# belinghy/SteppingStone

Measured on AMD Instinct MI355X. Metric: env-steps/sec (batched random-action rollout), higher is better.
Workload: dtype f32; 1 GPU; Walker3DStepperEnv-v0, 4096 envs per MI355X, curriculum 0 (flat terrain), on-device Philox U(-1,1) actions, auto-reset on; envs_total=4096, parallelism=env-shard x1, ranks=1, steps_per_launch=1000, prewarm_steps=256

## Files before the change

steppingstone_amd/csrc/ss_dynamics.hpp:

```cpp
#pragma once
#include "ss_math.hpp"
#include "ss_pair.hpp"

namespace ss {

constexpr float kH = 1.0f / 240.0f;
constexpr float kDt = 1.0f / 60.0f;
constexpr float kGrav = 9.8f;
constexpr float kPlankA = kStonePlankHalfLength, kPlankB = kStonePlankHalfWidth;
constexpr int kPgsIters = 5;
constexpr float kErp = 0.2f;
constexpr float kSlop = 0.001f;
constexpr float kVcorrMax = 2.0f;


constexpr int kWave = 64;
constexpr int kEnvsPerWave = 32;
constexpr int kLdsSlots = 40;
constexpr int kSlotsA = 20;
constexpr int kLdsC = 0;
constexpr int kLdsT = 18;
constexpr int kLdsHead = 36;
constexpr int kScalarBase = kSlotsA * kWave * 4;
constexpr int kRecWords = 9;
constexpr int kCholWords = 15 + 6;
constexpr int kHandJc = 0, kHandL0 = kHandJc + 8 * kRecWords, kHandLc = kHandL0 + kCholWords, kHandDet = 129, kHandAct = 146, kHandFloats = 158, kHandCs = kHandLc;
constexpr bool bias_offload(int helpers) { return helpers >= 3; }
constexpr bool spine_packed(int helpers) { return helpers >= 3; }
constexpr bool torques_paired(int helpers, bool kstep) { return helpers >= 3 && kstep; }
constexpr bool response_from_lds(int helpers, bool kstep) { return helpers >= 3 && kstep; }
constexpr int kHandBias = kHandJc;
static_assert(24 <= 3 * kRecWords, "biases fit the spine records' place");
constexpr int kHandRows = kHandJc + 3 * kRecWords;
constexpr int kHandRows3 = 160;
constexpr int kHandFloats3 = kHandRows3 + 40;
constexpr int kHandSlots3 = (kHandFloats3 + 3) / 4;
constexpr int hand_slots(int helpers) { return helpers >= 3 ? kHandSlots3 : (kHandFloats + 3) / 4; }
constexpr bool rows_offload(int helpers) { return helpers >= 3; }
constexpr int kHandSlots = (kHandFloats + 3) / 4;
static_assert(kLdsSlots + kHandSlots <= 80, "two helper-variant workgroups must fit the 160 KiB of a CU (16384 envs: 512 workgroups)");
static_assert(kHandRows + 40 <= kHandJc + 8 * kRecWords, "rows fit the leg records' place");
constexpr int kHandBase = kLdsSlots * kWave * 4;
constexpr int kFarWord0 = kHandLc;
constexpr int kFarBytes = (kHandBase + kFarWord0 * kWave) * 4;
static_assert(kFarBytes <= 65536, "every hand-off word beyond the offset field of the lane's own base goes through the far base");
constexpr bool hand_far(int idx) { return idx >= kFarWord0; }
constexpr int hand_far_offset(int idx) { return (idx - kFarWord0) * kWave * 4; }
constexpr int lds_bytes(int helpers) { return (kLdsSlots + hand_slots(helpers)) * kWave * 16; }
constexpr int hand_last_word(int helpers) { return hand_slots(helpers) * 4 - 1; }
static_assert(kHandFloats3 - 1 <= hand_last_word(3) && kHandFloats + 2 - 1 <= hand_last_word(1), "the words in use (one helper: + kHandOut2's two) are allocated");
static_assert(kFarBytes + (kWave - 1) * 4 + hand_far_offset(hand_last_word(1)) + 4 <= lds_bytes(1), "one helper: far base + largest word is inside the allocation");
static_assert(kFarBytes + (kWave - 1) * 4 + hand_far_offset(hand_last_word(3)) + 4 <= lds_bytes(3), "three helpers: far base + largest word is inside the allocation");
static_assert(hand_far_offset(kFarWord0) == 0 && hand_far_offset(hand_last_word(3)) < 65536 && hand_far_offset(hand_last_word(1)) < 65536,
              "every far offset fits the 16-bit offset field");
static_assert(hand_far_offset(1) - hand_far_offset(0) == 256 && hand_far_offset(hand_last_word(3)) / 256 <= 255,
              "far offsets are multiples of 256 B within ds_*2st64_b32's reach");
constexpr int NH = 12;
enum { S_ACT = 0, S_Q = 12, S_QD = 24, S_WLAM = 36, S_POS = 48, S_QUAT = 51, S_VW = 55, S_VV = 58, S_STP = 61, S_STN = 70,
       S_WKEY = 79, S_END = 80 };
static_assert(S_END <= (kLdsSlots - kSlotsA) * 4, "LDS scalar region overflow");
constexpr bool warm_in_lds(int helpers) { return helpers < 3; }
constexpr bool reset_pose_offload(int helpers, bool kstep) { return helpers >= 3 && kstep; }
constexpr int S_POSE = S_WLAM;
static_assert(!(reset_pose_offload(0, true) && warm_in_lds(0)) && !(reset_pose_offload(1, true) && warm_in_lds(1)) &&
              !(reset_pose_offload(2, true) && warm_in_lds(2)) && !(reset_pose_offload(3, true) && warm_in_lds(3)),
              "the reset pose lives where the warm-start impulses would: only a kernel that keeps those in registers has the words to spare");
static_assert(S_POSE + NH <= S_POS, "twelve words");

constexpr int kHalf[NH] = {0, 1, 2, 3, 4, 5, 6, 7, 13, 14, 15, 16};
constexpr int left_twin(int jr) { return jr < 3 ? jr : (jr < 8 ? jr + 5 : jr + 4); }
constexpr bool mirror_flips(int j) { return kAxis[j] != 1; }
__host__ __device__ constexpr float mirror_sign(int j, float m) { return mirror_flips(j) ? m : 1.f; }
__host__ __device__ constexpr float action_lane_sign(int jr, float m) {
  return jr < 3 ? mirror_sign(jr, m) : (float)kPolicySign[jr];
}
__host__ __device__ constexpr float policy_true_sign(int jr, int side) {
  return jr < 3 ? 1.f : (float)kPolicySign[jr] * ((mirror_flips(jr) && side) ? -1.f : 1.f);
}
constexpr int first_child_half(int b) {
  int r = -1;
  for (int i = 0; i < NH; ++i)
    if (kParent[kHalf[i]] == b) r = kHalf[i] + 1;
  return r;
}

#define SS_MEMBAR() asm volatile("" ::: "memory")
#if defined(__HIP_DEVICE_COMPILE__)
#define SS_WAVE_SYNC() asm volatile("" ::: "memory")
#else
#define SS_WAVE_SYNC() ss_host_wave_sync()
#endif

#if defined(SS_PROFILE_PHASES) && defined(__HIP_DEVICE_COMPILE__)
struct Prof { uint32_t t[16]; uint32_t last; };
#define SS_PROF_DECL Prof& prof,
#define SS_PROF_ARG prof,
#define SS_PROF_RAW(i) do { uint32_t _n = __builtin_amdgcn_readfirstlane((uint32_t)__builtin_amdgcn_s_memtime()); \
    prof.t[i] = __builtin_amdgcn_readfirstlane(prof.t[i] + (_n - __builtin_amdgcn_readfirstlane(prof.last))); prof.last = _n; } while (0)
#ifdef SS_PROFILE_EPILOGUE
#define SS_PROF(i) SS_PROF_RAW(0)
#define SS_PROFE(i) SS_PROF_RAW(i)
#else
#define SS_PROF(i) SS_PROF_RAW(i)
#define SS_PROFE(i) ((void)0)
#endif
#else
#define SS_PROFE(i) ((void)0)
struct Prof { int unused; };
#define SS_PROF_DECL
#define SS_PROF_ARG
#define SS_PROF(i) ((void)0)
#endif

#if defined(SS_FUZZ_SCHED) && defined(__HIP_DEVICE_COMPILE__)
__device__ __forceinline__ void ss_fuzz(uint32_t site) {
  uint32_t h = (uint32_t)__builtin_amdgcn_s_memtime() ^ (site * 0x9E3779B9u);
  h *= 0x85EBCA6Bu; h ^= h >> 13; h *= 0xC2B2AE35u; h ^= h >> 16;
  h = __builtin_amdgcn_readfirstlane(h);
  const uint32_t n = ((h >> 8) & 3u) == 0u ? (h & 255u) : (h & 15u);
#pragma unroll 1
// ... 5 lines not shown
#endif

constexpr bool cs_offload(int helpers) { return helpers >= 3; }

struct Lds {
  float* base;
  int lane;
  SSD float2& q2(int item) const { return reinterpret_cast<float2*>(base)[item * kWave + lane]; }
  SSD float& s(int idx) const { return base[kScalarBase + idx * kWave + lane]; }
  SSD float& hs(int idx) const {
#if defined(__HIP_DEVICE_COMPILE__)
    if (hand_far(idx)) {
      int off = kFarBytes + lane * 4;
      asm("" : "+v"(off));
      return *reinterpret_cast<float*>(reinterpret_cast<char*>(base) + off + hand_far_offset(idx));
    }
#endif
    return base[kHandBase + idx * kWave + lane];
  }
};

struct Stones {
  float p[3][3], nrm[3][3], tilt[3][2];
};

struct FootReport {
  int contact;
  int on_target;
  float sole[3];
};

struct Warm {
  float lam[4][3];
  int key;
};
SSD void warm_clear(Warm& w) {
#pragma unroll
  for (int k = 0; k < 4; ++k) w.lam[k][0] = w.lam[k][1] = w.lam[k][2] = 0.f;
  w.key = 0;
}

template <class T>
struct JRecT {
  T cs, sn, Uw[3], Uv[3], Dinv, u;
};
using JRec = JRecT<float>;
using JRec2 = JRecT<ssf2>;
static_assert(sizeof(JRec2) == 2 * sizeof(JRec), "a pair record is two scalar records, nothing else");
struct JointCache {
  JRec r[NH];
  Chol6 L0;
};
constexpr int half_pos(int j) { return j <= 7 ? j : j - 5; }
SSD void put_rec(const Lds& L, int k, const JRec& r) {
  L.hs(kHandJc + k * kRecWords + 0) = r.cs; L.hs(kHandJc + k * kRecWords + 1) = r.sn; L.hs(kHandJc + k * kRecWords + 2) = r.Dinv;
#pragma unroll
  for (int m = 0; m < 3; ++m) { L.hs(kHandJc + k * kRecWords + 3 + m) = r.Uw[m]; L.hs(kHandJc + k * kRecWords + 6 + m) = r.Uv[m]; }
}
SSD void get_rec(const Lds& L, int k, JRec& r) {
  r.cs = L.hs(kHandJc + k * kRecWords + 0); r.sn = L.hs(kHandJc + k * kRecWords + 1); r.Dinv = L.hs(kHandJc + k * kRecWords + 2);
#pragma unroll
  for (int m = 0; m < 3; ++m) { r.Uw[m] = L.hs(kHandJc + k * kRecWords + 3 + m); r.Uv[m] = L.hs(kHandJc + k * kRecWords + 6 + m); }
}
SSD void put_chol(const Lds& L, const Chol6& c) {
#pragma unroll
  for (int m = 0; m < 15; ++m) L.hs(kHandL0 + m) = c.l[m];
#pragma unroll
  for (int m = 0; m < 6; ++m) L.hs(kHandL0 + 15 + m) = c.di[m];
}
SSD void get_chol(const Lds& L, Chol6& c) {
#pragma unroll
  for (int i = 0; i < 15; ++i) c.l[i] = L.hs(kHandL0 + i);
#pragma unroll
  for (int i = 0; i < 6; ++i) c.di[i] = L.hs(kHandL0 + 15 + i);
}

SSD float xchg(float x) {
#if defined(__HIP_DEVICE_COMPILE__)
  return __builtin_bit_cast(float, __builtin_amdgcn_mov_dpp(__builtin_bit_cast(int, x), 0xB1, 0xF, 0xF, true));
#else
  return ss_host_xchg(x);
#endif
}
SSD uint32_t xchg_u32(uint32_t x) {
#if defined(__HIP_DEVICE_COMPILE__)
  return (uint32_t)__builtin_amdgcn_mov_dpp((int)x, 0xB1, 0xF, 0xF, true);
#else
  return __builtin_bit_cast(uint32_t, ss_host_xchg(__builtin_bit_cast(float, x)));
#endif
}
SSD int xchg_i(int x) {
#if defined(__HIP_DEVICE_COMPILE__)
  return __builtin_amdgcn_mov_dpp(x, 0xB1, 0xF, 0xF, true);
#else
  return (int)ss_host_xchg((float)x);
#endif
}
SSD SV mirror_sv(const SV& a) {
  SV o = {{-a.w[0], a.w[1], -a.w[2]}, {a.v[0], -a.v[1], a.v[2]}};
  return o;
}
SSD SV xchg_sv(const SV& a) {
  SV t;
#pragma unroll
  for (int i = 0; i < 3; ++i) { t.w[i] = xchg(a.w[i]); t.v[i] = xchg(a.v[i]); }
  return mirror_sv(t);
}
SSD ABI xchg_abi(const ABI& a) {
  ABI o;
  constexpr float sa[6] = {1.f, 1.f, 1.f, -1.f, 1.f, -1.f};
#pragma unroll
  for (int i = 0; i < 6; ++i) { o.A.m[i] = sa[i] * xchg(a.A.m[i]); o.C.m[i] = sa[i] * xchg(a.C.m[i]); }
  constexpr float sw[3] = {-1.f, 1.f, -1.f}, sv[3] = {1.f, -1.f, 1.f};
#pragma unroll
  for (int i = 0; i < 3; ++i)
#pragma unroll
// ... 309 lines not shown

template <class Model, int K>
SSD void row_moment(float (&w)[6]) {
  constexpr float cx = Model::corners[K][0], cy = Model::corners[K][1], cz = Model::corners[K][2];
  w[0] = cy * w[5] - cz * w[4];
  w[1] = cz * w[3] - cx * w[5];
  w[2] = cx * w[4] - cy * w[3];
}
template <class Model>
SSD void jacobian_rows(const DetectOut& det, const Lds& L, ssf2 (&rWp)[12][3], float (&rB)[4]) {
  const int active = det.active, cslot = det.cslot;
  const float (&Rf)[3][3] = det.Rf;
  const float (&pen)[4] = det.pen;
  static_for<0, 4>([&](auto Kc) {
    constexpr int k = decltype(Kc)::value;
    const bool on = (active >> k) & 1;
    const int sl = (cslot >> (2 * k)) & 3;
    float n[3];
#pragma unroll
    for (int i = 0; i < 3; ++i) n[i] = on ? L.s(S_STN + sl * 3 + i) : (i == 2 ? 1.f : 0.f);
    float t1[3] = {1.f - n[0] * n[0], -n[0] * n[1], -n[0] * n[2]};
    float inv = SS_RSQRT(t1[0] * t1[0] + t1[1] * t1[1] + t1[2] * t1[2]);
    t1[0] *= inv; t1[1] *= inv; t1[2] *= inv;
    float t2[3];
    cross(n, t1, t2);
    float corr = fmaxf(pen[k] - kSlop, 0.f);
    rB[k] = on ? fminf(kErp * corr * (1.0f / kH), kVcorrMax) : 0.f;
    static_for<0, 3>([&](auto Dc) {
      constexpr int d = decltype(Dc)::value, row = k * 3 + d;
      const float* dir = d == 0 ? n : (d == 1 ? t1 : t2);
      float w[6];
#pragma unroll
      for (int c = 0; c < 3; ++c) w[3 + c] = Rf[0][c] * dir[0] + Rf[1][c] * dir[1] + Rf[2][c] * dir[2];
      row_moment<Model, k>(w);
#pragma unroll
      for (int i = 0; i < 3; ++i) rWp[row][i] = ssf2{w[2 * i], w[2 * i + 1]};
    });
  });
}

template <class JT, class T>
SSD SVT<T> aba_acc(const JRecT<T>& r, const T& qd, const SVT<T>& aprev, const SVT<T>& vb, T& qdd) {
  constexpr int ax = JT::AX, ai = (ax + 1) % 3, aj = (ax + 2) % 3;
  SVT<T> a = xmotion<JT>(r.cs, r.sn, aprev);
  a.w[ai] += qd * vb.w[aj]; a.w[aj] -= qd * vb.w[ai];
  a.v[ai] += qd * vb.v[aj]; a.v[aj] -= qd * vb.v[ai];
  T dotv = r.Uw[0] * a.w[0] + r.Uw[1] * a.w[1] + r.Uw[2] * a.w[2] + r.Uv[0] * a.v[0] + r.Uv[1] * a.v[1] +
           r.Uv[2] * a.v[2];
  qdd = r.Dinv * (r.u - dotv);
  a.w[ax] += qdd;
  return a;
}

#ifndef SS_HOST_HARNESS
template <class Model, int HELPERS, int CS_PER, class Extra>
__device__ __forceinline__ void helper_substep(int helper, const Lds& L, Extra&& extra) {
  static_assert(CS_PER == 4 || CS_PER == 6, "the 12 cos / sin pairs go to three helpers (4 each) or to two (6 each)");
  __syncthreads();
  SS_FUZZ(0x10u + helper);
  if constexpr (cs_offload(HELPERS)) {
    constexpr int kIdle = HELPERS - NH / CS_PER;
    const int first = (helper - kIdle) * CS_PER;
    if (kIdle == 0 || helper >= kIdle) {
      float qh[CS_PER], c_[CS_PER], s_[CS_PER];
#pragma unroll
      for (int k = 0; k < CS_PER; ++k) qh[k] = L.s(S_Q + first + k);
      SS_MEMBAR();
#pragma unroll
      for (int k = 0; k < CS_PER; ++k) ss_sincos(qh[k], s_[k], c_[k]);
#pragma unroll
      for (int k = 0; k < CS_PER; ++k) { L.hs(kHandCs + first + k) = c_[k]; L.hs(kHandCs + NH + first + k) = s_[k]; }
    }
    __syncthreads();
    SS_FUZZ(0x20u + helper);
  }
  float rowdir[12][3], rowB[4];
  DetectOut det0;
  if (helper == 0) {
    float cs8[8], sn8[8];
    float quat[4] = {L.s(S_QUAT), L.s(S_QUAT + 1), L.s(S_QUAT + 2), L.s(S_QUAT + 3)};
    if constexpr (cs_offload(HELPERS)) {
#pragma unroll
      for (int k = 0; k < 8; ++k) { cs8[k] = L.hs(kHandCs + k); sn8[k] = L.hs(kHandCs + NH + k); }
      SS_MEMBAR();
    } else {
      float q8[8];
#pragma unroll
      for (int k = 0; k < 8; ++k) q8[k] = L.s(S_Q + k);
      SS_MEMBAR();
#pragma unroll
      for (int k = 0; k < 8; ++k) ss_sincos(q8[k], sn8[k], cs8[k]);
    }
    float Rb[3][3];
    quat_rot(quat, Rb);
    DetectOut det;
    FootReport fr;
    fk_detect<Model, (HELPERS < 3)>(cs8, sn8, Rb, L, det, fr);
    const int flags = det.active | (det.cslot << 4) | (fr.contact << 12) | (fr.on_target << 13);
    L.hs(kHandDet + 13) = __builtin_bit_cast(float, flags);
#pragma unroll
    for (int i = 0; i < 3; ++i) L.hs(kHandDet + 14 + i) = fr.sole[i];
    if constexpr (!rows_offload(HELPERS)) {
#pragma unroll
      for (int a = 0; a < 3; ++a)
#pragma unroll
        for (int c = 0; c < 3; ++c) L.hs(kHandDet + a * 3 + c) = det.Rf[a][c];
#pragma unroll
// ... 59 lines not shown
  static_for<0, 3>([&](auto Cc) {
    constexpr int c = decltype(Cc)::value;
    if (HELPERS == 1 || helper == c) {
      const LamPair lp = operator_pair_b<Model, c>(L, jc, oc[HELPERS == 1 ? c : 0]);
#pragma unroll
      for (int i = 0; i < 3; ++i) {
        L.hs(kHandLc + (2 * c) * 6 + 2 * i) = lp.a[i].x; L.hs(kHandLc + (2 * c) * 6 + 2 * i + 1) = lp.a[i].y;
        L.hs(kHandLc + (2 * c + 1) * 6 + 2 * i) = lp.b[i].x; L.hs(kHandLc + (2 * c + 1) * 6 + 2 * i + 1) = lp.b[i].y;
      }
    }
  });
  __syncthreads();
  SS_FUZZ(0x50u + helper);
}
#endif

template <class Model, int J>
SSD void joint_limit(float q, float& viol, float& kl, float& dl) {
  constexpr float lo = Model::lo[J], hi = Model::hi[J], klim = Model::klim[J], dlim = Model::dlim[J];
  static_assert(lo < hi, "a joint's range is not empty");
  viol = fminf(q - lo, 0.f) + fmaxf(q - hi, 0.f);
  uint32_t m = viol != 0.f ? 0xFFFFFFFFu : 0u;
  SS_REG(m);
  kl = __builtin_bit_cast(float, __builtin_bit_cast(uint32_t, klim) & m);
  dl = __builtin_bit_cast(float, __builtin_bit_cast(uint32_t, dlim) & m);
}

template <class Model, int J>
SSD void joint_tau(float power, float q, float qd, float act, float& tau, float& Dadd) {
  constexpr float h = kH;
  constexpr float kd = Model::damping[J], ks = Model::stiffness[J], arm = Model::armature[J], tq = Model::torque[J];
  float viol, kl, dl;
  joint_limit<Model, J>(q, viol, kl, dl);
  tau = power * tq * act - kd * qd - ks * (q + h * qd) - kl * (viol + h * qd) - dl * qd;
  Dadd = arm + h * (kd + dl) + (h * h) * (ks + kl);
}

template <class Model, int JL, int JA>
SSD void joint_tau(float power, ssf2 q, ssf2 qd, ssf2 act, ssf2& tau, ssf2& Dadd) {
  constexpr float h = kH;
  constexpr ssf2 kd = {Model::damping[JL], Model::damping[JA]}, ks = {Model::stiffness[JL], Model::stiffness[JA]};
  constexpr ssf2 arm = {Model::armature[JL], Model::armature[JA]}, tq = {Model::torque[JL], Model::torque[JA]};
  float violl, kll, dll, viola, kla, dla;
  joint_limit<Model, JL>(q.x, violl, kll, dll);
  joint_limit<Model, JA>(q.y, viola, kla, dla);
  const ssf2 viol = pkv(violl, viola), kl = pkv(kll, kla), dl = pkv(dll, dla);
  tau = power * tq * act - kd * qd - ks * (q + h * qd) - kl * (viol + h * qd) - dl * qd;
  Dadd = arm + h * (kd + dl) + (h * h) * (ks + kl);
}

template <class Model, int HELPERS = 0, bool KSTEP = false>
SSD void substep(SS_PROF_DECL float power, FootReport& fr, const Lds& L, Warm& wm) {
  constexpr float h = kH;
  JointCache jc;
#if defined(__HIP_DEVICE_COMPILE__)
  if constexpr (HELPERS > 0) { __syncthreads(); SS_FUZZ(0x1Fu); }
#endif
  SS_PROF(0);
  float qdfr[NH];
#define SS_QDF(k) qdfr[k]
  float qd_all[NH], q_all[NH], act_all[NH];
#pragma unroll
  for (int k = 0; k < NH; ++k) { q_all[k] = L.s(S_Q + k); qd_all[k] = L.s(S_QD + k); act_all[k] = L.s(S_ACT + k); }
  SS_MEMBAR();
  auto joint_tau = [&](auto Jc, float q, float qd, float act, float& tau, float& Dadd) {
    ss::joint_tau<Model, decltype(Jc)::value>(power, q, qd, act, tau, Dadd);
  };
  float tau_pre[NH], dadd_pre[NH];
  if constexpr (cs_offload(HELPERS) && HELPERS > 0) {
    static_for<0, NH>([&](auto Kc) {
      constexpr int k = decltype(Kc)::value;
      if constexpr (torques_paired(HELPERS, KSTEP) && k >= 3 && k != 7) {
        if constexpr (k < 7) {
          ssf2 tau2, dadd2;
          ss::joint_tau<Model, kHalf[k], kHalf[k + 5]>(power, pkv(q_all[k], q_all[k + 5]), pkv(qd_all[k], qd_all[k + 5]),
                                                       pkv(act_all[k], act_all[k + 5]), tau2, dadd2);
          tau_pre[k] = tau2.x; tau_pre[k + 5] = tau2.y; dadd_pre[k] = dadd2.x; dadd_pre[k + 5] = dadd2.y;
        }
      } else {
        joint_tau(std::integral_constant<int, kHalf[k]>{}, q_all[k], qd_all[k], act_all[k], tau_pre[k], dadd_pre[k]);
      }
    });
#if defined(__HIP_DEVICE_COMPILE__)
    __builtin_amdgcn_sched_barrier(0);
    SS_PROF(1);
    __syncthreads();
    SS_PROF(12);
    SS_FUZZ(0x2Fu);
    __builtin_amdgcn_sched_barrier(0);
#endif
#pragma unroll
    for (int k = 0; k < NH; ++k) { jc.r[k].cs = L.hs(kHandCs + k); jc.r[k].sn = L.hs(kHandCs + NH + k); }
    SS_MEMBAR();
  } else {
    static_for<0, NH>([&](auto Kc) {
      constexpr int k = decltype(Kc)::value;
      ss_sincos(q_all[k], jc.r[k].sn, jc.r[k].cs);
    });
  }
  auto tau_of = [&](auto Jc, auto Kc, float& tau, float& Dadd) {
    constexpr int k = decltype(Kc)::value;
    if constexpr (cs_offload(HELPERS) && HELPERS > 0) { tau = tau_pre[k]; Dadd = dadd_pre[k]; }
    else joint_tau(Jc, q_all[k], qd_all[k], act_all[k], tau, Dadd);
  };
  SS_PROF(1);

// ... 307 lines not shown
    det.cslot = (flags >> 4) & 255;
    fr.contact = (flags >> 12) & 1;
    fr.on_target = (flags >> 13) & 1;
#pragma unroll
    for (int i = 0; i < 3; ++i) fr.sole[i] = L.hs(kHandDet + 14 + i);
  } else {
    float cs8[8], sn8[8];
#pragma unroll
    for (int k = 0; k < 8; ++k) { cs8[k] = jc.r[k].cs; sn8[k] = jc.r[k].sn; }
    fk_detect<Model>(cs8, sn8, Rb, L, det, fr);
  }
  SS_PROF(6);

  float dqd[NH];
  SV dv0;
#pragma unroll
  for (int k = 0; k < NH; ++k) dqd[k] = 0.f;
#pragma unroll
  for (int i = 0; i < 3; ++i) { dv0.w[i] = 0.f; dv0.v[i] = 0.f; }
  const int active = det.active;
  const int pair_active = active | xchg_i(active);
  const bool in_contact = pair_active != 0;
  ssf2 Lc[6][3];
  SS_PROF(7);
  float V[6];
  ssf2 rWp[12][3];
  float rB[4];
  auto rows_free = [&]() {
      {
        SV a = v0f;
        static_for<0, 8>([&](auto Jc) {
          constexpr int j = decltype(Jc)::value;
          a = xmotion<Model, j>(jc.r[j].cs, jc.r[j].sn, a);
          a.w[kAxis[j]] += SS_QDF(j);
        });
#pragma unroll
        for (int i = 0; i < 3; ++i) { V[i] = a.w[i]; V[3 + i] = a.v[i]; }
      }
      if constexpr (!rows_offload(HELPERS)) jacobian_rows<Model>(det, L, rWp, rB);
      if constexpr (rows_offload(HELPERS)) {
        static_for<0, 12>([&](auto Rc) {
          constexpr int row = decltype(Rc)::value;
          float w[6];
#pragma unroll
          for (int i = 0; i < 3; ++i) w[3 + i] = L.hs(kHandRows3 + row * 3 + i);
          row_moment<Model, row / 3>(w);
#pragma unroll
          for (int i = 0; i < 3; ++i) rWp[row][i] = ssf2{w[2 * i], w[2 * i + 1]};
        });
#pragma unroll
        for (int k = 0; k < 4; ++k) rB[k] = L.hs(kHandRows3 + 36 + k);
      }
  };
  auto solve = [&]() {
      float ul[NH];
      float wlam_prev[4][3];
      int wkey_prev = 0;
      auto load_warm = [&]() {
        if constexpr (warm_in_lds(HELPERS)) {
          wkey_prev = __builtin_bit_cast(int, L.s(S_WKEY));
#pragma unroll
          for (int k = 0; k < 4; ++k)
#pragma unroll
            for (int d = 0; d < 3; ++d) wlam_prev[k][d] = L.s(S_WLAM + 3 * k + d);
        } else {
          wkey_prev = wm.key;
#pragma unroll
          for (int k = 0; k < 4; ++k)
#pragma unroll
            for (int d = 0; d < 3; ++d) wlam_prev[k][d] = wm.lam[k][d];
        }
      };
      if constexpr (HELPERS > 0) load_warm();
      if constexpr (HELPERS > 0) {
#pragma unroll
        for (int b = 0; b < 6; ++b)
#pragma unroll
          for (int i = 0; i < 3; ++i) Lc[b][i] = pkv(L.hs(kHandLc + b * 6 + 2 * i), L.hs(kHandLc + b * 6 + 2 * i + 1));
      }
      ssf2 rYp[12][3];
      float rIA[12];
      static_for<0, 12>([&](auto Rc) {
        constexpr int row = decltype(Rc)::value, k = row / 3;
        const bool on = (active >> k) & 1;
        ssf2 y[3];
#pragma unroll
        for (int i = 0; i < 3; ++i) y[i] = pk_mul_half<0>(Lc[0][i], rWp[row][0]);
        static_for<1, 6>([&](auto Bc) {
          constexpr int b = decltype(Bc)::value;
#pragma unroll
          for (int i = 0; i < 3; ++i) y[i] = pk_fma_half<b & 1>(Lc[b][i], rWp[row][b >> 1], y[i]);
        });
#pragma unroll
        for (int i = 0; i < 3; ++i) rYp[row][i] = y[i];
        ssf2 acc = rWp[row][0] * y[0];
        acc = rWp[row][1] * y[1] + acc;
        acc = rWp[row][2] * y[2] + acc;
        rIA[row] = on ? SS_RCP(acc.x + acc.y) : 0.f;
      });
      SS_PROF(8);
      if constexpr (HELPERS == 0) load_warm();
      float lam[4][3];
      const int key = active;
      int warm_any = 0;
#pragma unroll
      for (int k = 0; k < 4; ++k) {
        const bool w = ((active & wkey_prev) >> k) & 1;
        warm_any |= w ? 1 : 0;
// ... 68 lines not shown
        for (int l = 0; l < 6; ++l) {
          const float sc = (l & 1) ? dWo[l >> 1].y : dWo[l >> 1].x;
          const ssf2 s2 = {sc, sc};
#pragma unroll
          for (int i = 0; i < 3; ++i) {
            Vp[i] = Cc[l][i] * s2 + Vp[i];
          }
        }
      }
#if defined(__HIP_DEVICE_COMPILE__)
      if constexpr (response_from_lds(HELPERS, KSTEP)) {
        sweep_with([&](auto Rc) {
          constexpr int row = decltype(Rc)::value;
          if constexpr (row == 0 || row == 5 || row == 9) {
            __builtin_amdgcn_sched_barrier(0);
            if constexpr (row == 0) {
#pragma unroll
              for (int k = 7; k >= 5; --k) get_rec(L, k, jc.r[k]);
            } else if constexpr (row == 5) {
#pragma unroll
              for (int k = 4; k >= 0; --k) get_rec(L, k, jc.r[k]);
            } else {
              get_chol(L, jc.L0);
            }
            __builtin_amdgcn_sched_barrier(0);
          }
        });
      } else
#endif
      sweep();
      SV W = {{Wp[0].x, Wp[0].y, Wp[1].x}, {Wp[1].y, Wp[2].x, Wp[2].y}};
      if constexpr (warm_in_lds(HELPERS)) {
#pragma unroll
        for (int k = 0; k < 4; ++k)
#pragma unroll
          for (int d = 0; d < 3; ++d) L.s(S_WLAM + 3 * k + d) = lam[k][d];
        L.s(S_WKEY) = __builtin_bit_cast(float, key);
      } else {
#pragma unroll
        for (int k = 0; k < 4; ++k)
#pragma unroll
          for (int d = 0; d < 3; ++d) wm.lam[k][d] = lam[k][d];
        wm.key = key;
      }
      SS_PROF(9);
      {
        SV p = {{-W.w[0], -W.w[1], -W.w[2]}, {-W.v[0], -W.v[1], -W.v[2]}};
        static_rfor<7, 3>([&](auto Jc) { p = imp_up<Model, decltype(Jc)::value>(jc, ul, p); });
        const SV po = xchg_sv(p);
#pragma unroll
        for (int i = 0; i < 3; ++i) { p.w[i] += po.w[i]; p.v[i] += po.v[i]; }
        static_rfor<2, 0>([&](auto Jc) { p = imp_up<Model, decltype(Jc)::value>(jc, ul, p); });
        dv0 = chol6_solve_neg(jc.L0, p);
        SV d = dv0;
        static_for<0, 8>([&](auto Jc) {
          constexpr int j = decltype(Jc)::value;
          d = imp_down<Model, j, true>(jc, ul, d, &dqd[half_pos(j)]);
        });
        d = dv0;
        static_for<13, 17>([&](auto Jc) {
          constexpr int j = decltype(Jc)::value;
          d = imp_down<Model, j, false>(jc, ul, d, &dqd[half_pos(j)]);
        });
      }
  };
  if (!in_contact) {
    if constexpr (warm_in_lds(HELPERS)) L.s(S_WKEY) = 0.f;
    else wm.key = 0;
  }
  if constexpr (HELPERS == 0) {
    if (in_contact) {
      JointCache jo;
      operator_records_leg(jc, jo);
      operator_records_spine(jc, jo);
      static_for<0, 3>([&](auto Cc) { operator_T<Model, decltype(Cc)::value>(jo, L); });
      static_for<0, 3>([&](auto Cc) {
        constexpr int c = decltype(Cc)::value;
        OpCarry oc;
        operator_up<Model, c>(jo, oc);
        const LamPair lp = operator_pair_b<Model, c>(L, jo, oc);
#pragma unroll
        for (int i = 0; i < 3; ++i) { Lc[2 * c][i] = lp.a[i]; Lc[2 * c + 1][i] = lp.b[i]; }
      });
      rows_free();
      solve();
    }
  } else {
    if (in_contact) rows_free();
#if defined(__HIP_DEVICE_COMPILE__)
    SS_PROF(8);
    __syncthreads();
    SS_PROF(7);
    SS_FUZZ(0x5Fu);
#endif
    if (in_contact) solve();
  }
  SS_MEMBAR();
  SS_PROF(10);

  {
    float qf[NH], qq[NH];
#pragma unroll
    for (int k = 0; k < NH; ++k) { qf[k] = SS_QDF(k); qq[k] = L.s(S_Q + k); }
    SS_MEMBAR();
#pragma unroll
    for (int k = 0; k < NH; ++k) {
      float qd = qf[k] + dqd[k];
      L.s(S_QD + k) = qd;
      L.s(S_Q + k) = qq[k] + h * qd;
    }
  }
  SV v0n;
#pragma unroll
  for (int i = 0; i < 3; ++i) { v0n.w[i] = v0f.w[i] + dv0.w[i]; v0n.v[i] = v0f.v[i] + dv0.v[i]; }
#pragma unroll
  for (int i = 0; i < 3; ++i) { L.s(S_VW + i) = v0n.w[i]; L.s(S_VV + i) = v0n.v[i]; }
#pragma unroll
  for (int r = 0; r < 3; ++r)
    L.s(S_POS + r) += h * (Rb[r][0] * v0n.v[0] + Rb[r][1] * v0n.v[1] + Rb[r][2] * v0n.v[2]);
  {
    float qw = quat[0], qx = quat[1], qy = quat[2], qz = quat[3];
    float ox = v0n.w[0], oy = v0n.w[1], oz = v0n.w[2], hh = 0.5f * h;
    float nw = qw + hh * (-qx * ox - qy * oy - qz * oz);
    float nx = qx + hh * (qw * ox + qy * oz - qz * oy);
    float ny = qy + hh * (qw * oy - qx * oz + qz * ox);
    float nz = qz + hh * (qw * oz + qx * oy - qy * ox);
    float inv = SS_RSQRT(nw * nw + nx * nx + ny * ny + nz * nz);
    L.s(S_QUAT) = nw * inv; L.s(S_QUAT + 1) = nx * inv; L.s(S_QUAT + 2) = ny * inv; L.s(S_QUAT + 3) = nz * inv;
  }
  SS_MEMBAR();
  SS_PROF(11);
}

}
```

steppingstone_amd/csrc/ss_kernels.hpp:

```cpp
#pragma once
#include <cstdlib>

#include "ss_dynamics.hpp"
#include "../../include/steppingstone.h"

namespace ss {

enum { F_POS = 0, F_QUAT = 3, F_VEL = 7, F_Q = 13, F_QD = 34, F_POT = 55, F_ZINIT = 56, F_EPRET = 57, F_NNDR = 58,
       F_STONE = 59, F_HEAD = 59 + 24, F_EPRET_LO = 59 + 30, NF = 59 + 30 + 1 };
enum { I_N = 0, I_COUNT = 1, I_ELAPSED = 2, I_RNG = 3, I_FLAGS = 4, I_PROV = 5, NI = 6 };
constexpr int kNumStones = 20;
constexpr int kNumSubsteps = 4;
constexpr float kDeg = 0.017453292519943295f;

struct Knobs {
  const float* prob;
  int per_env_prob;
  int curriculum;
  float power;
  int auto_reset;
};

struct Params {
  float* fstate;
// ... 760 lines not shown
#else
      false;
#endif
  constexpr bool kPose =
#if defined(__HIP_DEVICE_COMPILE__)
      reset_pose_offload(HELPERS, ROLLOUT);
#else
      false;
#endif
  static_assert(!kPose || kOffload, "the pose's helper and the counter's hand-off word are the output stage's kernel's");
  const int e_raw = lane_global >> 1, side = lane_global & 1;
  const bool valid = e_raw < P.n;
  int e = valid ? e_raw : P.n - 1;
  const size_t np = (size_t)P.npad;
  const float m = side ? -1.f : 1.f;
  const Lds L{lds, lane};
  float ain[NH];
  load_in<!RANDOM_ACT>(P, e, RANDOM_ACT ? nullptr : io.act + (size_t)e * NJ, side, m, L, ain);

  const int nsteps = ROLLOUT ? io.nsteps : 1;
#pragma unroll 1
  for (int kstep = 0; kstep < nsteps; ++kstep) {
  SS_FUZZ(0x60u);
  if constexpr (RANDOM_ACT) {
    bool drawn = false;
    if constexpr (ROLLOUT && HELPERS > 1) {
      if (kstep > 0) {
        float a[NH];
#pragma unroll
        for (int k = 0; k < NH; ++k) a[k] = L.hs(kHandAct + k);
#pragma unroll
        for (int k = 0; k < NH; ++k) L.s(S_ACT + k) = a[k];
        drawn = true;
      }
    }
    if (!drawn) random_actions_half(P, e, side, m, (uint32_t)io.t + (uint32_t)kstep, [&](int k, float a) { L.s(S_ACT + k) = a; });
  } else {
    put_actions(L, m, ain);
  }

  const float power = P.knobs->power;
  FootReport fr;
#if defined(SS_PROFILE_PHASES) && defined(__HIP_DEVICE_COMPILE__)
  Prof prof;
#pragma unroll
  for (int i = 0; i < 16; ++i) prof.t[i] = 0;
  prof.last = (uint32_t)__builtin_amdgcn_s_memtime();
#endif
  Warm wm;
  warm_clear(wm);
  if constexpr (warm_in_lds(HELPERS)) L.s(S_WKEY) = 0.f;
#pragma unroll 1
  for (int k = 0; k < kNumSubsteps; ++k) substep<Model, HELPERS, ROLLOUT>(SS_PROF_ARG power, fr, L, wm);
  SS_FUZZ(0x61u);
  SS_PROF(12);
  SS_MEMBAR();
  SS_OPAQUE(e);
  const float* F = P.fstate + e;
  const Knobs K = *P.knobs;
  Cache c;
  load_cache(P, e, c);
  float pot_prev = F[F_POT * np], z_init = F[F_ZINIT * np];
  float ep_ret = F[F_EPRET * np], ep_lo = F[F_EPRET_LO * np], nn_dr = F[F_NNDR * np];
  int n = P.istate[e + I_N * np], count = P.istate[e + I_COUNT * np], elapsed = P.istate[e + I_ELAPSED * np];
  uint32_t ctr = (uint32_t)P.istate[e + I_RNG * np];
  const uint32_t ctr_in = ctr;
  SS_PROFE(1);

  float pos[3], quat[4];
  SV v0;
  get_base(L, m, pos, quat, v0);
  elapsed += 1;
  const float my_sole[3] = {fr.sole[0], m * fr.sole[1], fr.sole[2]};
  float ot_sole[3];
#pragma unroll
  for (int i = 0; i < 3; ++i) ot_sole[i] = xchg(my_sole[i]);
  const int ot_contact = xchg_i(fr.contact), ot_target = xchg_i(fr.on_target);
  float sole[2][3];
#pragma unroll
  for (int i = 0; i < 3; ++i) { sole[0][i] = side ? ot_sole[i] : my_sole[i]; sole[1][i] = side ? my_sole[i] : ot_sole[i]; }
  int flags = side ? (ot_contact | (fr.contact << 1)) : (fr.contact | (ot_contact << 1));
  const int on_target = fr.on_target | ot_target;
  SS_PROFE(2);
  float accv = 0.f, e_sum = 0.f, a2 = 0.f;
  int at_limit = 0;
  static_for<0, NH>([&](auto Kc) {
    constexpr int k = decltype(Kc)::value, jr = kHalf[k];
    constexpr float mid = 0.5f * (Model::lo[jr] + Model::hi[jr]);
    constexpr float span = Model::hi[jr] - Model::lo[jr];
    const float q = L.s(S_Q + k), qd = L.s(S_QD + k), a = L.s(S_ACT + k);
    const bool mine = (jr >= 3) || (side == 0);
    accv += q + qd;
    if (mine) {
      e_sum += fabsf(a * (0.1f * qd));
      a2 += a * a;
      if (fabsf(2.f * (q - mid) / span) > 0.99f) at_limit += 1;
    }
  });
  accv += pos[0] + pos[1] + pos[2] + quat[0] + quat[1] + quat[2] + quat[3];
#pragma unroll
  for (int i = 0; i < 3; ++i) accv += v0.w[i] + v0.v[i];
  e_sum += xchg(e_sum);
  a2 += xchg(a2);
  at_limit += xchg_i(at_limit);
  const bool finite = finite_bits(accv) && (xchg_i(finite_bits(accv) ? 1 : 0) != 0);
  SS_PROFE(3);
// ... 198 lines not shown
  SS_FUZZ(0x70u + wave);
  if (wave == 0) {
    step_env<Model, RANDOM_ACT, HELPERS>(P, io, blockIdx.x * kWave + lane, lane, lds);
  } else {
    const Lds L{lds, lane};
#pragma unroll 1
    for (int k = 0; k < kNumSubsteps; ++k) helper_substep<Model, HELPERS, 6>(wave - 1, L, [](int) {});
  }
}
template <class Model>
__global__ __launch_bounds__(kWave, 1) void rollout_kernel(Params P, StepIO io) {
  __shared__ float4 lds4[kLdsSlots * kWave];
  step_env<Model, true, 0, true>(P, io, blockIdx.x * kWave + threadIdx.x, threadIdx.x, reinterpret_cast<float*>(lds4));
}
template <class Model, int HELPERS>
__global__ __launch_bounds__(kWave * (1 + HELPERS), 1) void rollout_kernel_helped(Params P, StepIO io) {
  __shared__ float4 lds4[(kLdsSlots + hand_slots(HELPERS)) * kWave];
  const int wave = __builtin_amdgcn_readfirstlane(threadIdx.x >> 6), lane = threadIdx.x & (kWave - 1);
  float* lds = reinterpret_cast<float*>(lds4);
  SS_FUZZ(0x70u + wave);
  if (wave == 0) {
    step_env<Model, true, HELPERS, true>(P, io, blockIdx.x * kWave + lane, lane, lds);
  } else {
    const Lds L{lds, lane};
    const int lane_global = blockIdx.x * kWave + lane, side = lane_global & 1;
    const int e = min(lane_global >> 1, P.n - 1);
    const float m = side ? -1.f : 1.f;
    constexpr int kPoseHelper = 0;
    uint32_t ctr_pose = 0u;
    if constexpr (reset_pose_offload(HELPERS, true))
      if (wave - 1 == kPoseHelper) ctr_pose = (uint32_t)P.istate[e + I_RNG * (size_t)P.npad];
#pragma unroll 1
    for (int kstep = 0; kstep < io.nsteps; ++kstep)
#pragma unroll 1
      for (int k = 0; k < kNumSubsteps; ++k) {
        helper_substep<Model, HELPERS, 4>(wave - 1, L, [&](int helper) {
          if (k != 0) return;
          SS_FUZZ(0x80u + helper);
          constexpr int kActHelper = 1, kEmitHelper = HELPERS - 1;
          if (HELPERS > 1 && helper == kActHelper && kstep + 1 < io.nsteps)
            random_actions_half(P, e, side, m, (uint32_t)io.t + (uint32_t)kstep + 1u, [&](int j, float a) { L.hs(kHandAct + j) = a; });
          if (out_offload(HELPERS, true) && helper == kEmitHelper && kstep > 0) emit_from_handoff<Model, true>(P, io, L, lane, lane_global, kstep - 1, lds);
        });
        if constexpr (reset_pose_offload(HELPERS, true)) {
          if (k == 0 && wave - 1 == kPoseHelper) {
            SS_FUZZ(0xA0u);
            const uint32_t ctr_now = kstep == 0 ? ctr_pose : __builtin_bit_cast(uint32_t, L.hs(kHandCtr));
            if (kstep == 0 || __any(ctr_now != ctr_pose)) {
              ctr_pose = ctr_now;
              reset_pose_half<Model>(P, e, side, m, ctr_now, [&](int j, float q) { L.s(S_POSE + j) = q; });
            }
          }
        }
      }
    if constexpr (out_offload(HELPERS, true)) {
      __syncthreads();
      SS_FUZZ(0x90u + wave);
      if (wave == 2) emit_from_handoff<Model, true>(P, io, L, lane, lane_global, io.nsteps - 1, lds);
    }
  }
}

template <class Model>
SSD void reset_env(const Params& P, int e, float* obs_row) {
  const size_t np = (size_t)P.npad;
  Dyn s;
  Cache c;
  uint32_t ctr = (uint32_t)P.istate[e + I_RNG * np];
  float pot, z_init, nn_dr;
  env_reset<Model>(P, e, s, c, ctr, pot, z_init, nn_dr);
  store_dyn(P, e, s);
  store_cache(P, e, c);
  const float straight[3][2] = {{1.f, 0.f}, {1.f, 0.f}, {1.f, 0.f}};
  store_headings(P, e, straight);
  P.fstate[e + F_POT * np] = pot;
  P.fstate[e + F_ZINIT * np] = z_init;
  P.fstate[e + F_EPRET * np] = 0.f;
  P.fstate[e + F_EPRET_LO * np] = 0.f;
  P.fstate[e + F_NNDR * np] = nn_dr;
  P.istate[e + I_N * np] = 1;
  P.istate[e + I_COUNT * np] = 0;
  P.istate[e + I_ELAPSED * np] = 0;
  P.istate[e + I_RNG * np] = (int)ctr;
  P.istate[e + I_FLAGS * np] = 0;
  if (obs_row) {
    float o[SS_OBS_DIM];
    write_obs<Model>(s, z_init, 0, c, o);
#pragma unroll
    for (int i = 0; i < SS_OBS_DIM; ++i) obs_row[i] = o[i];
  }
}

template <class Model>
__global__ __launch_bounds__(kWave) void reset_kernel(Params P, float* obs) {
  const int e = blockIdx.x * kWave + threadIdx.x;
  if (e >= P.n) return;
  reset_env<Model>(P, e, obs ? obs + (size_t)e * SS_OBS_DIM : nullptr);
}

template <class Model>
__global__ __launch_bounds__(kWave) void obs_kernel(Params P, float* obs) {
  const int e = blockIdx.x * kWave + threadIdx.x;
  if (e >= P.n) return;
  const size_t np = (size_t)P.npad;
  Dyn s;
  Cache c;
// ... 51 lines not shown
```

Before: 99.36 million env-steps/s.

## Offload arm impulse response and base integration to helper waves

After the contact solve, the main wave hands off dv0, the four arm joint records and the free base velocity through LDS. Helper wave 1 then propagates the impulse down the arm chain and integrates the arm joints, while helper wave 2 integrates the base pose and velocity. This takes work off the main wave's critical path. In exchange it adds an extra __syncthreads per substep plus one after the last substep, along with LDS traffic for the handoff.

```diff
diff --git a/steppingstone_amd/csrc/ss_dynamics.hpp b/steppingstone_amd/csrc/ss_dynamics.hpp
--- a/steppingstone_amd/csrc/ss_dynamics.hpp
+++ b/steppingstone_amd/csrc/ss_dynamics.hpp
@@ -66,6 +66,19 @@
               !(reset_pose_offload(2, true) && warm_in_lds(2)) && !(reset_pose_offload(3, true) && warm_in_lds(3)),
               "the reset pose lives where the warm-start impulses would: only a kernel that keeps those in registers has the words to spare");
 static_assert(S_POSE + NH <= S_POS, "twelve words");
+#ifndef SS_ARM_TAIL
+#define SS_ARM_TAIL 1
+#endif
+#ifndef SS_BASE_TAIL
+#define SS_BASE_TAIL 1
+#endif
+constexpr bool arm_tail_offload(int helpers, bool kstep) { return SS_ARM_TAIL != 0 && helpers >= 3 && kstep; }
+constexpr bool base_tail_offload(int helpers, bool kstep) { return SS_BASE_TAIL != 0 && helpers >= 3 && kstep; }
+constexpr bool limb_tail_offload(int helpers, bool kstep) { return arm_tail_offload(helpers, kstep) || base_tail_offload(helpers, kstep); }
+constexpr int kHandArm = kHandRows3, kHandDv0 = kHandDet, kHandV0f = kHandDv0 + 6;
+constexpr int kArmHelper = 1, kBaseHelper = 2;
+static_assert(kHandArm + 4 * kRecWords <= kHandRows3 + 36, "the arm records fit the rows' directions");
+static_assert(kHandV0f + 6 <= kHandDet + 13, "dv0 and v0f stay below the detection's flags word and the sole");
 
 constexpr int kHalf[NH] = {0, 1, 2, 3, 4, 5, 6, 7, 13, 14, 15, 16};
 constexpr int left_twin(int jr) { return jr < 3 ? jr : (jr < 8 ? jr + 5 : jr + 4); }
@@ -177,16 +190,18 @@
   Chol6 L0;
 };
 constexpr int half_pos(int j) { return j <= 7 ? j : j - 5; }
-SSD void put_rec(const Lds& L, int k, const JRec& r) {
-  L.hs(kHandJc + k * kRecWords + 0) = r.cs; L.hs(kHandJc + k * kRecWords + 1) = r.sn; L.hs(kHandJc + k * kRecWords + 2) = r.Dinv;
-#pragma unroll
-  for (int m = 0; m < 3; ++m) { L.hs(kHandJc + k * kRecWords + 3 + m) = r.Uw[m]; L.hs(kHandJc + k * kRecWords + 6 + m) = r.Uv[m]; }
-}
-SSD void get_rec(const Lds& L, int k, JRec& r) {
-  r.cs = L.hs(kHandJc + k * kRecWords + 0); r.sn = L.hs(kHandJc + k * kRecWords + 1); r.Dinv = L.hs(kHandJc + k * kRecWords + 2);
-#pragma unroll
-  for (int m = 0; m < 3; ++m) { r.Uw[m] = L.hs(kHandJc + k * kRecWords + 3 + m); r.Uv[m] = L.hs(kHandJc + k * kRecWords + 6 + m); }
-}
+SSD void put_rec_at(const Lds& L, int w, const JRec& r) {
+  L.hs(w + 0) = r.cs; L.hs(w + 1) = r.sn; L.hs(w + 2) = r.Dinv;
+#pragma unroll
+  for (int m = 0; m < 3; ++m) { L.hs(w + 3 + m) = r.Uw[m]; L.hs(w + 6 + m) = r.Uv[m]; }
+}
+SSD void get_rec_at(const Lds& L, int w, JRec& r) {
+  r.cs = L.hs(w + 0); r.sn = L.hs(w + 1); r.Dinv = L.hs(w + 2);
+#pragma unroll
+  for (int m = 0; m < 3; ++m) { r.Uw[m] = L.hs(w + 3 + m); r.Uv[m] = L.hs(w + 6 + m); }
+}
+SSD void put_rec(const Lds& L, int k, const JRec& r) { put_rec_at(L, kHandJc + k * kRecWords, r); }
+SSD void get_rec(const Lds& L, int k, JRec& r) { get_rec_at(L, kHandJc + k * kRecWords, r); }
 SSD void put_chol(const Lds& L, const Chol6& c) {
 #pragma unroll
   for (int m = 0; m < 15; ++m) L.hs(kHandL0 + m) = c.l[m];
@@ -602,7 +617,74 @@
   return a;
 }
 
+template <class Model>
+SSD void arm_response(const JointCache& jc, const SV& dv0, float* dqd) {
+  SV d = dv0;
+  static_for<13, 17>([&](auto Jc) {
+    constexpr int j = decltype(Jc)::value;
+    d = imp_down<Model, j, false>(jc, nullptr, d, &dqd[half_pos(j)]);
+  });
+}
+SSD void integrate_joint(const Lds& L, int k, float qf, float dqd, float qq) {
+  constexpr float h = kH;
+  float qd = qf + dqd;
+  L.s(S_QD + k) = qd;
+  L.s(S_Q + k) = qq + h * qd;
+}
+SSD void integrate_base(const Lds& L, const SV& v0f, const SV& dv0, const float (&Rb)[3][3], const float (&quat)[4]) {
+  constexpr float h = kH;
+  SV v0n;
+#pragma unroll
+  for (int i = 0; i < 3; ++i) { v0n.w[i] = v0f.w[i] + dv0.w[i]; v0n.v[i] = v0f.v[i] + dv0.v[i]; }
+#pragma unroll
+  for (int i = 0; i < 3; ++i) { L.s(S_VW + i) = v0n.w[i]; L.s(S_VV + i) = v0n.v[i]; }
+#pragma unroll
+  for (int r = 0; r < 3; ++r)
+    L.s(S_POS + r) += h * (Rb[r][0] * v0n.v[0] + Rb[r][1] * v0n.v[1] + Rb[r][2] * v0n.v[2]);
+  {
+    float qw = quat[0], qx = quat[1], qy = quat[2], qz = quat[3];
+    float ox = v0n.w[0], oy = v0n.w[1], oz = v0n.w[2], hh = 0.5f * h;
+    float nw = qw + hh * (-qx * ox - qy * oy - qz * oz);
+    float nx = qx + hh * (qw * ox + qy * oz - qz * oy);
+    float ny = qy + hh * (qw * oy - qx * oz + qz * ox);
+    float nz = qz + hh * (qw * oz + qx * oy - qy * ox);
+    float inv = SS_RSQRT(nw * nw + nx * nx + ny * ny + nz * nz);
+    L.s(S_QUAT) = nw * inv; L.s(S_QUAT + 1) = nx * inv; L.s(S_QUAT + 2) = ny * inv; L.s(S_QUAT + 3) = nz * inv;
+  }
+}
+
 #ifndef SS_HOST_HARNESS
+template <class Model>
+__device__ __forceinline__ void helper_arm_tail(const Lds& L) {
+  const int active = __builtin_bit_cast(int, L.hs(kHandDet + 13)) & 15;
+  JointCache jc;
+#pragma unroll
+  for (int i = 0; i < 4; ++i) get_rec_at(L, kHandArm + i * kRecWords, jc.r[8 + i]);
+  SV dv0;
+#pragma unroll
+  for (int i = 0; i < 3; ++i) { dv0.w[i] = L.hs(kHandDv0 + i); dv0.v[i] = L.hs(kHandDv0 + 3 + i); }
+  float qf[NH], qq[NH], dqd[NH];
+#pragma unroll
+  for (int k = 8; k < NH; ++k) { qf[k] = L.s(S_QD + k); qq[k] = L.s(S_Q + k); dqd[k] = 0.f; }
+  SS_MEMBAR();
+  const bool in_contact = (active | xchg_i(active)) != 0;
+  if (in_contact) arm_response<Model>(jc, dv0, dqd);
+#pragma unroll
+  for (int k = 8; k < NH; ++k) integrate_joint(L, k, qf[k], dqd[k], qq[k]);
+}
+__device__ __forceinline__ void helper_base_tail(const Lds& L) {
+  float quat[4] = {L.s(S_QUAT), L.s(S_QUAT + 1), L.s(S_QUAT + 2), L.s(S_QUAT + 3)};
+  SV v0f, dv0;
+#pragma unroll
+  for (int i = 0; i < 3; ++i) {
+    dv0.w[i] = L.hs(kHandDv0 + i); dv0.v[i] = L.hs(kHandDv0 + 3 + i);
+    v0f.w[i] = L.hs(kHandV0f + i); v0f.v[i] = L.hs(kHandV0f + 3 + i);
+  }
+  SS_MEMBAR();
+  float Rb[3][3];
+  quat_rot(quat, Rb);
+  integrate_base(L, v0f, dv0, Rb, quat);
+}
 template <class Model, int HELPERS, int CS_PER, class Extra>
 __device__ __forceinline__ void helper_substep(int helper, const Lds& L, Extra&& extra) {
   static_assert(CS_PER == 4 || CS_PER == 6, "the 12 cos / sin pairs go to three helpers (4 each) or to two (6 each)");
@@ -768,6 +850,12 @@
 template <class Model, int HELPERS = 0, bool KSTEP = false>
 SSD void substep(SS_PROF_DECL float power, FootReport& fr, const Lds& L, Warm& wm) {
   constexpr float h = kH;
+#if defined(__HIP_DEVICE_COMPILE__)
+  constexpr bool kArmTail = arm_tail_offload(HELPERS, KSTEP), kBaseTail = base_tail_offload(HELPERS, KSTEP);
+#else
+  constexpr bool kArmTail = false, kBaseTail = false;
+#endif
+  constexpr bool kTail = kArmTail || kBaseTail;
   JointCache jc;
 #if defined(__HIP_DEVICE_COMPILE__)
   if constexpr (HELPERS > 0) { __syncthreads(); SS_FUZZ(0x1Fu); }
@@ -1181,8 +1269,16 @@
         for (int k = 0; k < 4; ++k) rB[k] = L.hs(kHandRows3 + 36 + k);
       }
   };
+  float ul[NH];
+  auto respond_down = [&]() {
+      SV d = dv0;
+      static_for<0, 8>([&](auto Jc) {
+        constexpr int j = decltype(Jc)::value;
+        d = imp_down<Model, j, true>(jc, ul, d, &dqd[half_pos(j)]);
+      });
+      if constexpr (!kArmTail) arm_response<Model>(jc, dv0, dqd);
+  };
   auto solve = [&]() {
-      float ul[NH];
       float wlam_prev[4][3];
       int wkey_prev = 0;
       auto load_warm = [&]() {
@@ -1357,16 +1453,7 @@
         for (int i = 0; i < 3; ++i) { p.w[i] += po.w[i]; p.v[i] += po.v[i]; }
         static_rfor<2, 0>([&](auto Jc) { p = imp_up<Model, decltype(Jc)::value>(jc, ul, p); });
         dv0 = chol6_solve_neg(jc.L0, p);
-        SV d = dv0;
-        static_for<0, 8>([&](auto Jc) {
-          constexpr int j = decltype(Jc)::value;
-          d = imp_down<Model, j, true>(jc, ul, d, &dqd[half_pos(j)]);
-        });
-        d = dv0;
-        static_for<13, 17>([&](auto Jc) {
-          constexpr int j = decltype(Jc)::value;
-          d = imp_down<Model, j, false>(jc, ul, d, &dqd[half_pos(j)]);
-        });
+        if constexpr (!kTail) respond_down();
       }
   };
   if (!in_contact) {
@@ -1393,46 +1480,49 @@
   } else {
     if (in_contact) rows_free();
 #if defined(__HIP_DEVICE_COMPILE__)
+    if constexpr (kArmTail) {
+#pragma unroll
+      for (int i = 0; i < 4; ++i) put_rec_at(L, kHandArm + i * kRecWords, jc.r[8 + i]);
+#pragma unroll
+      for (int k = 8; k < NH; ++k) L.s(S_QD + k) = SS_QDF(k);
+    }
+    if constexpr (kBaseTail) {
+#pragma unroll
+      for (int i = 0; i < 3; ++i) { L.hs(kHandV0f + i) = v0f.w[i]; L.hs(kHandV0f + 3 + i) = v0f.v[i]; }
+    }
     SS_PROF(8);
     __syncthreads();
     SS_PROF(7);
     SS_FUZZ(0x5Fu);
 #endif
     if (in_contact) solve();
+#if defined(__HIP_DEVICE_COMPILE__)
+    if constexpr (kTail) {
+#pragma unroll
+      for (int i = 0; i < 3; ++i) { L.hs(kHandDv0 + i) = dv0.w[i]; L.hs(kHandDv0 + 3 + i) = dv0.v[i]; }
+      __builtin_amdgcn_sched_barrier(0);
+      SS_PROF(10);
+      __syncthreads();
+      SS_PROF(6);
+      SS_FUZZ(0xBFu);
+      __builtin_amdgcn_sched_barrier(0);
+      if (in_contact) respond_down();
+    }
+#endif
   }
   SS_MEMBAR();
   SS_PROF(10);
 
   {
+    constexpr int kMine = kArmTail ? 8 : NH;
     float qf[NH], qq[NH];
 #pragma unroll
-    for (int k = 0; k < NH; ++k) { qf[k] = SS_QDF(k); qq[k] = L.s(S_Q + k); }
+    for (int k = 0; k < kMine; ++k) { qf[k] = SS_QDF(k); qq[k] = L.s(S_Q + k); }
     SS_MEMBAR();
 #pragma unroll
-    for (int k = 0; k < NH; ++k) {
-      float qd = qf[k] + dqd[k];
-      L.s(S_QD + k) = qd;
-      L.s(S_Q + k) = qq[k] + h * qd;
-    }
-  }
-  SV v0n;
-#pragma unroll
-  for (int i = 0; i < 3; ++i) { v0n.w[i] = v0f.w[i] + dv0.w[i]; v0n.v[i] = v0f.v[i] + dv0.v[i]; }
-#pragma unroll
-  for (int i = 0; i < 3; ++i) { L.s(S_VW + i) = v0n.w[i]; L.s(S_VV + i) = v0n.v[i]; }
-#pragma unroll
-  for (int r = 0; r < 3; ++r)
-    L.s(S_POS + r) += h * (Rb[r][0] * v0n.v[0] + Rb[r][1] * v0n.v[1] + Rb[r][2] * v0n.v[2]);
-  {
-    float qw = quat[0], qx = quat[1], qy = quat[2], qz = quat[3];
-    float ox = v0n.w[0], oy = v0n.w[1], oz = v0n.w[2], hh = 0.5f * h;
-    float nw = qw + hh * (-qx * ox - qy * oy - qz * oz);
-    float nx = qx + hh * (qw * ox + qy * oz - qz * oy);
-    float ny = qy + hh * (qw * oy - qx * oz + qz * ox);
-    float nz = qz + hh * (qw * oz + qx * oy - qy * ox);
-    float inv = SS_RSQRT(nw * nw + nx * nx + ny * ny + nz * nz);
-    L.s(S_QUAT) = nw * inv; L.s(S_QUAT + 1) = nx * inv; L.s(S_QUAT + 2) = ny * inv; L.s(S_QUAT + 3) = nz * inv;
-  }
+    for (int k = 0; k < kMine; ++k) integrate_joint(L, k, qf[k], dqd[k], qq[k]);
+  }
+  if constexpr (!kBaseTail) integrate_base(L, v0f, dv0, Rb, quat);
   SS_MEMBAR();
   SS_PROF(11);
 }
diff --git a/steppingstone_amd/csrc/ss_kernels.hpp b/steppingstone_amd/csrc/ss_kernels.hpp
--- a/steppingstone_amd/csrc/ss_kernels.hpp
+++ b/steppingstone_amd/csrc/ss_kernels.hpp
@@ -836,6 +836,13 @@
   if constexpr (warm_in_lds(HELPERS)) L.s(S_WKEY) = 0.f;
 #pragma unroll 1
   for (int k = 0; k < kNumSubsteps; ++k) substep<Model, HELPERS, ROLLOUT>(SS_PROF_ARG power, fr, L, wm);
+#if defined(__HIP_DEVICE_COMPILE__)
+  if constexpr (limb_tail_offload(HELPERS, ROLLOUT)) {
+    SS_PROF(11);
+    __syncthreads();
+    SS_FUZZ(0xCFu);
+  }
+#endif
   SS_FUZZ(0x61u);
   SS_PROF(12);
   SS_MEMBAR();
@@ -1140,6 +1147,18 @@
             }
           }
         }
+        if constexpr (limb_tail_offload(HELPERS, true)) {
+          __syncthreads();
+          SS_FUZZ(0xB0u + (wave - 1));
+          if constexpr (arm_tail_offload(HELPERS, true))
+            if (wave - 1 == kArmHelper) helper_arm_tail<Model>(L);
+          if constexpr (base_tail_offload(HELPERS, true))
+            if (wave - 1 == kBaseHelper) helper_base_tail(L);
+          if (k == kNumSubsteps - 1) {
+            __syncthreads();
+            SS_FUZZ(0xC0u + (wave - 1));
+          }
+        }
       }
     if constexpr (out_offload(HELPERS, true)) {
       __syncthreads();
```

After: 103.4 million env-steps/s, median of 6. 1.04x the previous value.
